# EmilyJrxx/YOLO_PPF_Pose_Estimation

Measured on AMD Instinct MI355X. Metric: PPF pair-matches/sec (accumulator votes) per cropped scene, higher is better.
Workload: dtype u32 votes / f64 pair features

## Files before the change

### yolo_ppf_pose_estimation_amd/csrc/ppf_match_kernels.h

```cpp
#ifndef PPF_MATCH_KERNELS_H
#define PPF_MATCH_KERNELS_H

#ifndef PPF_GUARD_REL
#define PPF_GUARD_REL 5e-7f
#endif
#ifndef PPF_AGG_MIN_HITS
#define PPF_AGG_MIN_HITS 24
#endif
#ifndef PPF_AGG_MIN_RECORDS
#define PPF_AGG_MIN_RECORDS 32
#endif
#ifndef PPF_ABL_COUNTED
#define PPF_ABL_COUNTED 1
#endif
#ifndef PPF_ABL_OWNCELL
#define PPF_ABL_OWNCELL 1
#endif
#ifndef PPF_ABL_DIRECT_SMALL
#define PPF_ABL_DIRECT_SMALL 1
#endif
#ifndef PPF_ABL_DIRECT_BIG
#define PPF_ABL_DIRECT_BIG 1
#endif
#ifndef PPF_MOCK_PAIRBINS
// ... 24 lines not shown
#ifndef PPF_COST_TABLE
#define PPF_COST_TABLE 16
#endif
#ifndef PPF_COST_MIN_HITS
#define PPF_COST_MIN_HITS 8
#endif
#ifndef PPF_COST_ITEM
#define PPF_COST_ITEM 512
#endif
#ifndef PPF_ACC32_COST
#define PPF_ACC32_COST 1.02
#endif
#ifndef PPF_ACC32_SWITCH
#define PPF_ACC32_SWITCH 0.05
#endif
#ifndef PPF_TWO_QUEUES
#define PPF_TWO_QUEUES 0
#endif
#ifndef PPF_PIPE_VALU
#define PPF_PIPE_VALU 4
#endif

constexpr int PAIR_BLOCK = 256;
#ifndef PPF_PAIRS_PER_THREAD
#define PPF_PAIRS_PER_THREAD 12
#endif
constexpr int PAIRS_PER_THREAD = PPF_PAIRS_PER_THREAD;
constexpr int VOTE_BLOCK = 1024;
constexpr int VOTE_WAVES = VOTE_BLOCK / 64;
constexpr int VOTE_UNROLL = 4;
constexpr int VOTE_CHUNK = 64 * VOTE_UNROLL * 4;
constexpr int VOTE_MAX_HITS = PPF_AGG_MIN_HITS;
#ifndef PPF_AGG_CHUNK
#define PPF_AGG_CHUNK 1024
#endif
static_assert(PPF_AGG_CHUNK >= 32 && PPF_AGG_CHUNK % 32 == 0, "chunks of pair records start in different blocks of 32 (MatchArgs::grp_hdr)");
constexpr int AGG_CHUNK = PPF_AGG_CHUNK;
constexpr int AGG_NY = 16;
constexpr int AGG_SUB = 191;
constexpr int AGG_MAX_ANGLES = 31;
#ifndef PPF_RUN_SEG
#define PPF_RUN_SEG 704
#endif
constexpr int RUN_SEG = PPF_RUN_SEG;
constexpr int RUN_SEG_MAX = 1024;
static_assert(RUN_SEG % 64 == 0 && RUN_SEG <= RUN_SEG_MAX && RUN_SEG_MAX == 1024, "the staging area is sized in steps of 64 runs");
constexpr int GROUP_BLOCK = 512;
#ifndef PPF_GROUP_MLP
#define PPF_GROUP_MLP 4
#endif
constexpr int GROUP_MLP = PPF_GROUP_MLP;
constexpr int GROUP_MAX_BUCKETS = 36000;
constexpr int POOL_STRIPES = 64;
constexpr int LDS_HEADER = 256;

constexpr int CUR_STRIDE = 32;
constexpr int CUR_SORTED = POOL_STRIPES * CUR_STRIDE;
constexpr int CUR_RUNS = CUR_SORTED + CUR_STRIDE;
constexpr int CUR_ODDVALUES = CUR_RUNS + CUR_STRIDE;
constexpr int CUR_OVFCOUNT = CUR_ODDVALUES + CUR_STRIDE;
constexpr int CUR_TABLES = CUR_OVFCOUNT + CUR_STRIDE;
constexpr int CUR_OVERFLOW = CUR_TABLES + CUR_STRIDE;
constexpr int CUR_WORDS = CUR_OVERFLOW + CUR_STRIDE;

constexpr int AGG_ROW = 20;
constexpr int AGG_ROW_CE = 17;
constexpr int AGG_SCRATCH = ((AGG_Q + 1) * AGG_ROW + 15) / 16 * 16;
constexpr int AGG_OFF_COLS = (AGG_Q + 1) * AGG_ROW;
constexpr uint32_t AGG_COLS_ALL = (2u << AGG_NY) - 1u;
constexpr int AGG_GROUP_CELLS = 4;
constexpr uint32_t AGG_NARROW_MAX = 255u / AGG_GROUP_CELLS;
constexpr uint32_t AGG_COLS_NARROW = 1u << 31;
constexpr uint32_t AGG_CELLS_FREE = (uint32_t)AGG_Q * 0x01010101u;
constexpr uint32_t AGG_GROUP_X = 8u;
static_assert(AGG_OFF_COLS % 4 == 0 && AGG_OFF_COLS + 4 <= AGG_SCRATCH, "the column mask lives in the padding behind the rows");
constexpr int TBL_OFF_A32 = AGG_SCRATCH;
constexpr int TBL_A32_BYTES = (AGG_NY * AGG_Q > 768 ? AGG_NY * AGG_Q : 768);
constexpr int TBL_OFF_IDX = TBL_OFF_A32 + TBL_A32_BYTES;
constexpr int TBL_BYTES = TBL_OFF_IDX + 192;
constexpr int AGG_OFF_CE = TBL_BYTES;
constexpr int TBL_BUILD_BYTES = AGG_OFF_CE + ((AGG_Q + 1) * 4 + 15) / 16 * 16;
static_assert(AGG_SUB * 4 <= 768 && AGG_SUB <= 192 && AGG_SUB < 256, "table hit range too long");
static_assert(AGG_SCRATCH % 16 == 0 && TBL_BYTES % 16 == 0, "tables are copied 16 bytes at a time");
constexpr int TABLE_BLOCK = 256;
constexpr double TBL_FRAC_MAX = 1.0 / PPF_AGG_MIN_HITS + 1.0 / AGG_SUB;
constexpr double TBL_FRAC_START = 0.02;

__device__ __forceinline__ float acos32_estimate(double x) {
  const double ax = ppf_fabs(x);
  const float xf = (float)ax;
  const float t = fmaxf((float)(1.0 - ax), 0.0f);
  float p = -0.001441536471247673f;
  p = __builtin_fmaf(p, xf, 0.007245631422847509f);
  p = __builtin_fmaf(p, xf, -0.01780921407043934f);
  p = __builtin_fmaf(p, xf, 0.03133561089634895f);
  p = __builtin_fmaf(p, xf, -0.0503128282725811f);
  p = __builtin_fmaf(p, xf, 0.08899927139282227f);
  p = __builtin_fmaf(p, xf, -0.21459989249706268f);
  p = __builtin_fmaf(p, xf, 1.5707963705062866f);
  const float a = __builtin_amdgcn_sqrtf(t) * p;
  return x >= 0.0 ? a : 3.14159274101257324f - a;
}

struct FastKeyConsts {
  float rstep32;
  float gq;
  double rdstep;
};

__device__ __forceinline__ void pair_key(const ppf_vec3& p1, const ppf_vec3& n1, const ppf_vec3& p2, const ppf_vec3& n2,
                                         const double angle_step, const double dist_step, const FastKeyConsts& fk, int32_t (&k)[4]) {
  const double dx = p2.x - p1.x, dy = p2.y - p1.y, dz = p2.z - p1.z;
  const double d2 = __builtin_fma(dz, dz, __builtin_fma(dy, dy, dx * dx));
  const double hd = 0.5 * d2;
  double rinv = __builtin_amdgcn_rsq(d2);
  rinv = rinv * __builtin_fma(-(hd * rinv), rinv, 1.5);
  rinv = rinv * __builtin_fma(-(hd * rinv), rinv, 1.5);
  const double f3 = d2 * rinv;
  const double x0 = __builtin_fma(n1.z, dz, __builtin_fma(n1.y, dy, n1.x * dx)) * rinv;
  const double x1 = __builtin_fma(n2.z, dz, __builtin_fma(n2.y, dy, n2.x * dx)) * rinv;
  const double x2 = __builtin_fma(n1.z, n2.z, __builtin_fma(n1.y, n2.y, n1.x * n2.x));
  bool slow = !(f3 > 2.0 * PPF_EPS) || !(ppf_fabs(x0) <= 1.0 - 1e-12) || !(ppf_fabs(x1) <= 1.0 - 1e-12) || !(ppf_fabs(x2) <= 1.0);
  {
    const float q0 = acos32_estimate(x0) * fk.rstep32, q1 = acos32_estimate(x1) * fk.rstep32,
                q2 = acos32_estimate(x2) * fk.rstep32;
    k[0] = (int)q0; k[1] = (int)q1; k[2] = (int)q2;
    const float lim = 0.5f - fk.gq;
    slow |= (__builtin_fabsf(__builtin_amdgcn_fractf(q0) - 0.5f) > lim) |
            (__builtin_fabsf(__builtin_amdgcn_fractf(q1) - 0.5f) > lim) |
            (__builtin_fabsf(__builtin_amdgcn_fractf(q2) - 0.5f) > lim);
    const double q3 = f3 * fk.rdstep;
    k[3] = (int)q3;
    const double fr3 = q3 - (double)k[3];
    slow |= !(fr3 > 1e-9 && fr3 < 1.0 - 1e-9) || !(q3 < 1.0e5);
  }
  if (slow) {
    double f[4] = {0, 0, 0, 0};
    ppf_pair_feature(p1, n1, p2, n2, f);
    k[0] = ppf_d2i(f[0] / angle_step); k[1] = ppf_d2i(f[1] / angle_step); k[2] = ppf_d2i(f[2] / angle_step);
    k[3] = ppf_d2i(f[3] / dist_step);
  }
}

__device__ __forceinline__ bool pair_key_darboux(const ppf_vec3& p1, const ppf_vec3& n1, const ppf_vec3& p2, const ppf_vec3& n2,
                                                 const double angle_step, const double dist_step, int32_t (&k)[4]) {
  double f[4];
  if (!ppf_pair_feature_darboux(p1, n1, p2, n2, f)) return false;
  k[0] = ppf_floor_key(f[0] / angle_step); k[1] = ppf_floor_key(f[1] / angle_step); k[2] = ppf_floor_key(f[2] / angle_step);
  k[3] = ppf_floor_key(f[3] / dist_step);
  return true;
}

struct MatchArgs {
  CloudSoA surf;
  CloudSoA paired;
  int same_cloud;
  int scene_step, ref_offset, ref_stride;
  int ref_base, n_ref;
  const SlotWord* slotmap;
  uint32_t slot_mask;
  const int32_t* key_lut;
  KeyDims kd;
  const uint32_t* bucket_off;
  int n_buckets;
  const uint4* records;
  int n_tiles, tile_refs, num_angles, n_model;
// ... 718 lines not shown
  const uint32_t before = (quarter >= 1 ? t1 : 0u) + (quarter >= 2 ? t2 : 0u) + (quarter >= 3 ? t3 : 0u);
  const uint32_t tot = __shfl(before + run, 3, 4);
#pragma unroll
  for (int t = 0; t < PER; t++) {
    less[t] += before;
    more[t] = tot - less[t] - c[t];
  }
  const int yy = lane >> 2;
  uint32_t colw;
  {
    unsigned long long o = __ballot(tot != 0u) & 0x1111111111111111ull;
    o = (o | (o >> 3)) & 0x0303030303030303ull;
    o = (o | (o >> 6)) & 0x000F000F000F000Full;
    o = (o | (o >> 12)) & 0x000000FF000000FFull;
    o = (o | (o >> 24)) & 0xFFFFull;
    colw = ((uint32_t)o | ((uint32_t)o << 1)) & AGG_COLS_ALL;
  }
  uint32_t cmax = 0;
#pragma unroll
  for (int t = 0; t < PER; t++) {
    const uint32_t mprev = __shfl_up(more[t], 4);
    const uint32_t v = less[t] + (lane >= 4 ? mprev : 0u);
    const uint32_t p = (uint32_t)(quarter * PER + t);
    lds_st8(ws + p * AGG_ROW + yy, v);
    if (yy == AGG_NY - 1) lds_st8(ws + p * AGG_ROW + AGG_NY, more[t]);
    cmax = max(cmax, yy == AGG_NY - 1 ? max(v, more[t]) : v);
  }
#pragma unroll
  for (int o = 32; o > 0; o >>= 1) cmax = max(cmax, (uint32_t)__shfl_xor((int)cmax, o));
  if (lane == 0) lds_st(ws + AGG_OFF_COLS, colw | (cmax <= AGG_NARROW_MAX ? AGG_COLS_NARROW : 0u));
  wave_lds_fence();
  uint32_t h = lane < AGG_Q ? lds_ld(ws + AGG_OFF_CE + lane * 4) : 0u;
#pragma unroll
  for (int o = 1; o < AGG_Q; o <<= 1) {
    const uint32_t y = __shfl_up(h, o);
    if (lane >= o) h += y;
  }
  wave_lds_fence();
  if (lane < AGG_Q) lds_st(ws + AGG_OFF_CE + lane * 4, h);
  if (lane == 0) lds_st(ws + AGG_OFF_CE + AGG_Q * 4, (uint32_t)ms);
  wave_lds_fence();
#pragma unroll
  for (int t = 0; t < 3; t++) {
    if (cell[t] != 0xFFFFu) {
      const uint32_t pos = lds_add_rtn(ws + AGG_OFF_CE + (cell[t] % (uint32_t)AGG_Q) * 4, 0xFFFFFFFFu) - 1u;
      lds_st(ws + TBL_OFF_A32 + pos * 4, a32[t]);
      lds_st8(ws + TBL_OFF_IDX + pos, (uint32_t)(lane + 64 * t));
    }
  }
  wave_lds_fence();
  if (lane < AGG_Q) {
    const uint2 se = lds_ld2(ws + AGG_OFF_CE + lane * 4);
    lds_st8(ws + lane * AGG_ROW + AGG_ROW_CE, se.x);
    lds_st8(ws + lane * AGG_ROW + AGG_ROW_CE + 1, se.y);
  }
  if (lane == 0) lds_st8(ws + AGG_Q * AGG_ROW + AGG_ROW_CE + 1, (uint32_t)ms);
  wave_lds_fence();
}

__device__ __forceinline__ float vote_guard_band(const int A) {
#ifdef PPF_FORCE_EXACT
  (void)A;
  return 1.0f;
#else
  return PPF_GUARD_REL * (float)A;
#endif
}

__global__ __launch_bounds__(TABLE_BLOCK) void k_tables(MatchArgs a) {
  __shared__ __align__(16) unsigned char tsm[(TABLE_BLOCK / 64) * TBL_BUILD_BYTES];
  const int lane = threadIdx.x & 63;
  const int wave = __builtin_amdgcn_readfirstlane(threadIdx.x >> 6);
  const uint32_t t = blockIdx.x * (TABLE_BLOCK / 64) + (uint32_t)wave;
  if (t >= a.table_cap) return;
  const uint2 d = a.table_desc[t];
  if (d.y == 0u) return;
  const uint32_t ws = (uint32_t)(uintptr_t)(lds_byte*)(tsm + wave * TBL_BUILD_BYTES);
  const int A = a.num_angles;
  const double s64 = (double)A / (4 * PPF_PI);
  const float S = (float)s64, Og = (float)(0.5 * (double)A + (double)vote_guard_band(A));
  table_build(ws, S, Og, s64, a.s_a64 + d.x, (int)d.y, lane);
  const lds_u32x4* src = (const lds_u32x4*)(uintptr_t)ws;
  uint4* __restrict__ dst = reinterpret_cast<uint4*>(a.tables + (size_t)t * TBL_BYTES);
  for (int q = lane; q < TBL_BYTES / 16; q += 64) {
    const u32x4_t v = src[q];
    dst[q] = make_uint4(v.x, v.y, v.z, v.w);
  }
}

__device__ __forceinline__ void agg_cell(const AggConsts& k, const float am, int& X, int& q) {
  const float x = __builtin_fmaf(am, k.S, k.half_a);
  X = (int)x;
  const float qf = __builtin_amdgcn_fractf(x) * (float)AGG_Q;
  q = (int)qf;
  const float fq = __builtin_amdgcn_fractf(qf);
  constexpr float band = 4.7e-6f * (float)AGG_Q;
  const bool near = !(fq > band && fq < 1.0f - band);
  bool one_by_one = am < -3.1415925f;
  if (__builtin_expect(__any(near), 0)) {
    if (near) {
      const double xd = (double)am * k.s64 + k.half_a64;
      const double Xd = __builtin_floor(xd);
      const double qd = (xd - Xd) * (double)AGG_Q;
      const double qfl = __builtin_floor(qd);
      const double fqd = qd - qfl;
      X = (int)Xd;
      q = (int)qfl;
      one_by_one |= !(fqd > 1e-7 && fqd < 1.0 - 1e-7);
    }
  }
  q = one_by_one ? AGG_Q : min(q, AGG_Q - 1);
}

__device__ uint32_t agg_cell_bits(const float am, const int A) {
  if (A > AGG_MAX_ANGLES) return 0u;
  AggConsts k;
  k.s64 = (double)A / (4 * PPF_PI);
  k.S = (float)k.s64;
  k.half_a = 0.5f * (float)A;
  k.half_a64 = 0.5 * (double)A;
  int X, q;
  agg_cell(k, am, X, q);
  return ((uint32_t)X << ROW_X_SHIFT) | ((uint32_t)q << ROW_Q_SHIFT);
}

struct __attribute__((packed, aligned(4))) gl_quad_t { uint32_t x, y, z, w; };
__device__ __forceinline__ uint4 gl_ld4(const uint32_t* __restrict__ p) {
  const gl_quad_t q = *reinterpret_cast<const gl_quad_t*>(p);
  return make_uint4(q.x, q.y, q.z, q.w);
}
__device__ __forceinline__ uint4 gl_ld4_at(const uint32_t* __restrict__ base, const uint32_t w) {
  return gl_ld4(reinterpret_cast<const uint32_t*>(reinterpret_cast<const char*>(base) + w * 4u));
}

__device__ __forceinline__ void agg_own_vote(const AggConsts& k, const uint32_t rz, const uint32_t rw, const float am_a, const float am_b,
                                             const uint32_t oa, const uint32_t ob, const bool da, const bool db, const uint32_t pa,
                                             const uint32_t pb, const uint32_t inc_a, const uint32_t inc_b,
                                             const unsigned char* __restrict__ tbl, const double* __restrict__ g_a64, const uint32_t ha,
                                             const uint32_t hb) {
  const float xa = __builtin_fmaf(am_a, k.S, __uint_as_float(oa)), xb = __builtin_fmaf(am_b, k.S, __uint_as_float(ob));
  int ba = (int)xa, bb = (int)xb;
  const float fa = da ? __builtin_amdgcn_fractf(xa) : 1.0f, fb = db ? __builtin_amdgcn_fractf(xb) : 1.0f;
  if (__builtin_expect(__any(__builtin_fminf(fa, fb) < k.G2), 0)) {
    uint32_t za = rz, zb = rw;
    asm volatile("" : "+v"(za), "+v"(zb));
    if (fa < k.G2) ba = vote_bin_exact_4pi(__uint_as_float(za), g_a64[tbl[TBL_OFF_IDX + ha]], k.A);
    if (fb < k.G2) bb = vote_bin_exact_4pi(__uint_as_float(zb), g_a64[tbl[TBL_OFF_IDX + hb]], k.A);
  }
  if (da) vote_one(pa, ba, inc_a);
  if (db) vote_one(pb, bb, inc_b);
}

struct AggOwn {
  uint32_t wa, wb;
  uint4 oa, ob;
};
__device__ __forceinline__ void agg_own_fetch(const AggConsts& k, const uint4 rec, const unsigned char* __restrict__ tbl, const int ms, AggOwn& o) {
  (void)ms;
  const uint32_t qa = (rec.x >> ROW_Q_SHIFT) & ROW_Q_MASK, qb = (rec.y >> ROW_Q_SHIFT) & ROW_Q_MASK;
  o.wa = lds_ld(k.ws + qa * AGG_ROW + 16);
  o.wb = lds_ld(k.ws + qb * AGG_ROW + 16);
#if PPF_ABL_OWNCELL
  const uint32_t* __restrict__ toff = reinterpret_cast<const uint32_t*>(tbl + TBL_OFF_A32);
  o.oa = gl_ld4_at(toff, __builtin_amdgcn_ubfe(o.wa, 8u, 8u));
  o.ob = gl_ld4_at(toff, __builtin_amdgcn_ubfe(o.wb, 8u, 8u));
#else
  (void)tbl;
#endif
}

__device__ __forceinline__ void agg_cast(const AggConsts& k, const uint32_t va, const uint32_t vb, const bool ha, const bool hb,
                                         const uint32_t (&wa)[5], const uint32_t (&wb)[5], const uint32_t cols) {
  uint32_t sa[4], sb[4];
  {
    const uint32_t sa0 = ha ? k.sel_hi : k.sel_lo, sta = ha ? k.step_hi : k.step_lo;
    const uint32_t sb0 = hb ? k.sel_hi : k.sel_lo, stb = hb ? k.step_hi : k.step_lo;
#pragma unroll
    for (int jj = 0; jj < 4; jj++) { sa[jj] = sa0 + (uint32_t)jj * sta; sb[jj] = sb0 + (uint32_t)jj * stb; }
  }
#if PPF_MOCK_PAIRBINS == 3
  {
    (void)cols;
    const uint32_t va8 = va & ~7u, vb8 = vb & ~7u;
#pragma unroll
    for (int j = 0; j <= AGG_NY; j += 2) {
      const int j1 = j + 1 > AGG_NY ? j : j + 1;
      const unsigned long long da = ((unsigned long long)__builtin_amdgcn_perm(0u, wa[j1 >> 2], sa[j1 & 3]) << 32) | __builtin_amdgcn_perm(0u, wa[j >> 2], sa[j & 3]);
      const unsigned long long db = ((unsigned long long)__builtin_amdgcn_perm(0u, wb[j1 >> 2], sb[j1 & 3]) << 32) | __builtin_amdgcn_perm(0u, wb[j >> 2], sb[j & 3]);
      typedef __attribute__((address_space(3))) unsigned long long lds_u64;
      (void)__hip_atomic_fetch_add((lds_u64*)(uintptr_t)(va8 + (uint32_t)((AGG_NY - j) * 4)), da, __ATOMIC_RELAXED, __HIP_MEMORY_SCOPE_WORKGROUP);
      (void)__hip_atomic_fetch_add((lds_u64*)(uintptr_t)(vb8 + (uint32_t)((AGG_NY - j) * 4)), db, __ATOMIC_RELAXED, __HIP_MEMORY_SCOPE_WORKGROUP);
    }
  }
#elif PPF_MOCK_PAIRBINS
  (void)cols;
#pragma unroll
  for (int j = 0; j <= AGG_NY; j += 2) {
    lds_add(va + (uint32_t)((AGG_NY - j) * 2), __builtin_amdgcn_perm(wa[(j + 1 > AGG_NY ? j : j + 1) >> 2], wa[j >> 2], sa[(j >> 1) & 3]));
    lds_add(vb + (uint32_t)((AGG_NY - j) * 2), __builtin_amdgcn_perm(wb[(j + 1 > AGG_NY ? j : j + 1) >> 2], wb[j >> 2], sb[(j >> 1) & 3]));
  }
#else
  uint32_t cm = cols;
  asm volatile("" : "+s"(cm));
  if (cm == AGG_COLS_ALL) {
#pragma unroll
    for (int j = 0; j <= AGG_NY; j++) {
      lds_add(va + (uint32_t)((AGG_NY - j) * 4), __builtin_amdgcn_perm(0u, wa[j >> 2], sa[j & 3]));
      lds_add(vb + (uint32_t)((AGG_NY - j) * 4), __builtin_amdgcn_perm(0u, wb[j >> 2], sb[j & 3]));
    }
  } else {
#pragma unroll
    for (int j = 0; j <= AGG_NY; j++) {
      if (cm & (1u << j)) {
        lds_add(va + (uint32_t)((AGG_NY - j) * 4), __builtin_amdgcn_perm(0u, wa[j >> 2], sa[j & 3]));
        lds_add(vb + (uint32_t)((AGG_NY - j) * 4), __builtin_amdgcn_perm(0u, wb[j >> 2], sb[j & 3]));
      }
    }
  }
#endif
}

__device__ __forceinline__ void agg_row_add(const uint32_t t, uint32_t (&w)[5]) {
  const uint2 r01 = lds_ld2(t), r23 = lds_ld2(t + 8);
  const uint32_t r4 = lds_ld(t + 16);
  w[0] += r01.x; w[1] += r01.y; w[2] += r23.x; w[3] += r23.y; w[4] += r4 & 0xFFu;
}

__device__ __forceinline__ void agg_group_pair(const AggConsts& k, const uint4 g, const uint32_t cols) {
  static_assert(AGG_GROUP_CELLS == 4, "a group record holds four cell bytes");
  const int Xa = (int)((g.x >> ROW_X_SHIFT) & 31u), Xb = (int)((g.y >> ROW_X_SHIFT) & 31u);
  const uint32_t pa = k.acc_base + (g.x & ROW_OFFSET_MASK), pb = k.acc_base + (g.y & ROW_OFFSET_MASK);
  const bool ha = (g.x & 1u) != 0, hb = (g.y & 1u) != 0;
  uint32_t va = pa + (uint32_t)((Xa - 8) * 4), vb = pb + (uint32_t)((Xb - 8) * 4);
  asm volatile("" : "+v"(va), "+v"(vb));
  uint32_t wa[5] = {0u, 0u, 0u, 0u, 0u}, wb[5] = {0u, 0u, 0u, 0u, 0u};
  agg_row_add(k.ws + (g.z & 0xFFu) * AGG_ROW, wa);
  agg_row_add(k.ws + (g.w & 0xFFu) * AGG_ROW, wb);
  agg_row_add(k.ws + __builtin_amdgcn_ubfe(g.z, 8u, 8u) * AGG_ROW, wa);
  agg_row_add(k.ws + __builtin_amdgcn_ubfe(g.w, 8u, 8u) * AGG_ROW, wb);
  if (__any(((g.z >> 16) != (AGG_CELLS_FREE >> 16)) | ((g.w >> 16) != (AGG_CELLS_FREE >> 16)))) {
    agg_row_add(k.ws + __builtin_amdgcn_ubfe(g.z, 16u, 8u) * AGG_ROW, wa);
    agg_row_add(k.ws + __builtin_amdgcn_ubfe(g.w, 16u, 8u) * AGG_ROW, wb);
    if (__any(((g.z >> 24) != (AGG_CELLS_FREE >> 24)) | ((g.w >> 24) != (AGG_CELLS_FREE >> 24)))) {
      agg_row_add(k.ws + (g.z >> 24) * AGG_ROW, wa);
      agg_row_add(k.ws + (g.w >> 24) * AGG_ROW, wb);
    }
  }
  agg_cast(k, va, vb, ha, hb, wa, wb, cols);
}

template <bool COUNTED>
__device__ __forceinline__ void agg_pair(const AggConsts& k, const uint4 rec, const AggOwn& own, const unsigned char* __restrict__ tbl,
                                         const double* __restrict__ g_a64, const uint32_t cols, uint32_t& votes, const bool live = true) {
  const float am_a = __uint_as_float(rec.z), am_b = __uint_as_float(rec.w);
  const uint32_t a4 = own.wa, b4 = own.wb;
  const uint2 ca = make_uint2(__builtin_amdgcn_ubfe(a4, 8u, 8u), __builtin_amdgcn_ubfe(a4, 16u, 8u));
  const uint2 cb = make_uint2(__builtin_amdgcn_ubfe(b4, 8u, 8u), __builtin_amdgcn_ubfe(b4, 16u, 8u));
  const uint32_t pa = k.acc_base + (rec.x & ROW_OFFSET_MASK), pb = k.acc_base + (rec.y & ROW_OFFSET_MASK);
  const uint32_t inc_a = vote_inc(k.vi, rec.x), inc_b = vote_inc(k.vi, rec.y);
#if !PPF_ABL_COUNTED
  (void)cols;
#else
  if constexpr (COUNTED) {
    const int Xa = (int)((rec.x >> ROW_X_SHIFT) & 31u), qa = (int)((rec.x >> ROW_Q_SHIFT) & ROW_Q_MASK);
    const int Xb = (int)((rec.y >> ROW_X_SHIFT) & 31u), qb = (int)((rec.y >> ROW_Q_SHIFT) & ROW_Q_MASK);
    const uint32_t ta = k.ws + (uint32_t)qa * AGG_ROW, tb = k.ws + (uint32_t)qb * AGG_ROW;
    const uint2 a01 = lds_ld2(ta), a23 = lds_ld2(ta + 8);
    const uint2 b01 = lds_ld2(tb), b23 = lds_ld2(tb + 8);
    const bool ha = (rec.x & 1u) != 0, hb = (rec.y & 1u) != 0;
    uint32_t va = pa + (uint32_t)((Xa - 8) * 4), vb = pb + (uint32_t)((Xb - 8) * 4);
    asm volatile("" : "+v"(va), "+v"(vb));
    const uint32_t wa[5] = {a01.x, a01.y, a23.x, a23.y, a4}, wb[5] = {b01.x, b01.y, b23.x, b23.y, b4};
    agg_cast(k, va, vb, ha, hb, wa, wb, cols);
  }
#endif
  const uint32_t na = live ? ca.y - ca.x : 0u, nb = live ? cb.y - cb.x : 0u;
  votes += na + nb;
#if PPF_ABL_OWNCELL
  if (__any((na > 0u) | (nb > 0u))) {
#define PPF_OWN_VOTE(OA, OB, J) \
    agg_own_vote(k, rec.z, rec.w, am_a, am_b, OA, OB, (J) < na, (J) < nb, pa, pb, inc_a, inc_b, tbl, g_a64, ca.x + (J), cb.x + (J))
    PPF_OWN_VOTE(own.oa.x, own.ob.x, 0u);
    if (__any((1u < na) | (1u < nb))) {
      PPF_OWN_VOTE(own.oa.y, own.ob.y, 1u);
      if (__any((2u < na) | (2u < nb))) {
        PPF_OWN_VOTE(own.oa.z, own.ob.z, 2u);
        if (__any((3u < na) | (3u < nb))) {
          PPF_OWN_VOTE(own.oa.w, own.ob.w, 3u);
          if (__builtin_expect(__any((4u < na) | (4u < nb)), 0)) {
            const uint32_t* __restrict__ toff = reinterpret_cast<const uint32_t*>(tbl + TBL_OFF_A32);
            for (uint32_t done = 4u;;) {
              const uint4 oa = gl_ld4_at(toff, min(ca.x + done, (uint32_t)AGG_SUB)), ob = gl_ld4_at(toff, min(cb.x + done, (uint32_t)AGG_SUB));
              PPF_OWN_VOTE(oa.x, ob.x, done + 0u);
              if (!__any((done + 1u < na) | (done + 1u < nb))) break;
              PPF_OWN_VOTE(oa.y, ob.y, done + 1u);
              if (!__any((done + 2u < na) | (done + 2u < nb))) break;
              PPF_OWN_VOTE(oa.z, ob.z, done + 2u);
              if (!__any((done + 3u < na) | (done + 3u < nb))) break;
              PPF_OWN_VOTE(oa.w, ob.w, done + 3u);
              done += 4u;
              if (!__any((done < na) | (done < nb))) break;
            }
          }
        }
      }
    }
#undef PPF_OWN_VOTE
  }
#endif
}

constexpr int ITEM_C_BITS = 13, ITEM_NH_BITS = 8;
static_assert(VOTE_CHUNK < (1 << ITEM_C_BITS) && AGG_CHUNK < (1 << ITEM_C_BITS) && VOTE_MAX_HITS < (1 << ITEM_NH_BITS) && AGG_SUB < (1 << ITEM_NH_BITS),
              "an item's records and hits share one word of its staged record");
__host__ __device__ constexpr size_t vote_seg_bytes(int run_seg) { return ((size_t)(run_seg + 1) * 24 + 15) / 16 * 16; }
__host__ __device__ constexpr int vote_item_seg(int run_seg) { return (int)(vote_seg_bytes(run_seg) / 16); }
struct VoteItem {
  const uint4* src;
  uint32_t c;
  uint32_t g0;
  int nh;
  bool agg;
  double a64;
  uint4 rec0;
  const unsigned char* tbl;
};

#ifndef PPF_PREFETCH
#define PPF_PREFETCH 2
#endif
__device__ __forceinline__ void vote_fetch_hits(VoteItem& it, const int lane, const MatchArgs& a) {
  it.a64 = (!it.agg && lane < it.nh) ? a.s_a64[it.g0 + lane] : 0.0;
}
__device__ __forceinline__ void vote_fetch_records(VoteItem& it, const int lane) {
  const uint32_t idx = (!it.agg && it.c <= 32) ? ((uint32_t)lane >> 1) : (uint32_t)lane;
  it.rec0 = rec_at(it.src, min(idx, it.c - 1));
}
static_assert(AGG_SCRATCH / 16 <= 128, "the table copy gives a lane two 16-byte pieces");

__device__ __forceinline__ void vote_item_settle(VoteItem& it) {
  uint32_t lo = (uint32_t)__double2loint(it.a64), hi = (uint32_t)__double2hiint(it.a64);
  asm volatile("" : "+v"(lo), "+v"(hi), "+v"(it.rec0.x), "+v"(it.rec0.y), "+v"(it.rec0.z), "+v"(it.rec0.w));
  it.a64 = __hiloint2double((int)hi, (int)lo);
}

struct VoteRun {
  uint32_t off, cnt;
  uint32_t hit0, m;
  uint32_t tbl0;
  uint32_t nchunk;
  uint32_t agg;
};
__device__ __forceinline__ uint4 vote_item_record(const VoteRun& r, const uint32_t sub, const uint32_t chunk) {
  const uint32_t chunk_sz = r.agg ? (uint32_t)AGG_CHUNK : (uint32_t)VOTE_CHUNK;
  const uint32_t group_sz = r.agg ? (uint32_t)AGG_SUB : (uint32_t)VOTE_MAX_HITS;
  const uint32_t c = min(chunk_sz, r.cnt - chunk * chunk_sz), nh = min(group_sz, r.m - sub * group_sz);
  return make_uint4(r.off + chunk * chunk_sz, r.hit0 + sub * group_sz, r.tbl0 + sub, c | (nh << ITEM_C_BITS) | (r.agg << (ITEM_C_BITS + ITEM_NH_BITS)));
}

__device__ __forceinline__ void vote_locate(VoteItem& it, const uint32_t item, const uint4* seg, const int lane, const MatchArgs& a,
                                            const uint4* __restrict__ records) {
  const uint4 rec = seg[item];
  const uint32_t first = (uint32_t)__builtin_amdgcn_readfirstlane((int)rec.x);
  const uint32_t w = (uint32_t)__builtin_amdgcn_readfirstlane((int)rec.w);
  it.g0 = (uint32_t)__builtin_amdgcn_readfirstlane((int)rec.y);
  it.agg = (w >> (ITEM_C_BITS + ITEM_NH_BITS)) != 0;
  it.c = w & ((1u << ITEM_C_BITS) - 1u);
  it.nh = (int)((w >> ITEM_C_BITS) & ((1u << ITEM_NH_BITS) - 1u));
  it.src = records + first;
  it.tbl = it.agg ? a.tables + (size_t)(uint32_t)__builtin_amdgcn_readfirstlane((int)rec.z) * TBL_BYTES : nullptr;
#if PPF_PREFETCH >= 1
  vote_fetch_hits(it, lane, a);
#endif
#if PPF_PREFETCH >= 2
  vote_fetch_records(it, lane);
// ... 14 lines not shown
  uint32_t* acc = lds_acc + GW;

  const int tid = threadIdx.x, lane = tid & 63;
  const int wave = __builtin_amdgcn_readfirstlane(tid >> 6);
  const bool listed = ACC32 && a.acc32 == 2;
  const uint32_t n_work = listed ? 2u * a.cursors[CUR_OVFCOUNT] : gridDim.x;
  uint32_t wid = blockIdx.x;
  if (ACC32 && wid >= n_work) return;
  do {
  int vt, tile, r;
  if (listed) {
    const uint32_t e = a.ovf_list[wid >> 1];
    r = (int)(e & 0xFFFFu);
    tile = (int)(e >> 16);
    vt = 2 * tile + (int)(wid & 1u);
  } else {
    vt = (int)(wid / (uint32_t)a.n_ref);
    tile = ACC32 ? vt >> 1 : vt;
    r = (int)a.perm[wid - (uint32_t)vt * (uint32_t)a.n_ref];
  }
  const int rg = a.ref_base + r;
  const int tile_base = tile * a.tile_refs;
  const int refs_here = min(a.tile_refs, a.n_model - tile_base);
  const int H = (a.tile_refs + 1) >> 1;
  const int words = GW + min(H, refs_here) * P + 1;
  constexpr bool acc32 = ACC32;
  if (tid == 0) { red[50] = red[51] = red[52] = red[53] = red[58] = red[59] = 0u; }

  const uint32_t* __restrict__ boff = a.bucket_off + (size_t)tile * (a.n_buckets + 1);
  if (!ACC32 && a.item_votes) {
    unsigned long long v = 0;
    for (int blk = 0; blk < a.n_rounds; blk++) {
      const uint2 rb = a.run_blocks[(size_t)r * a.n_rounds + blk];
      for (uint32_t i = (uint32_t)tid; i < rb.y; i += VOTE_BLOCK) {
        const uint4 run = a.runs[rb.x + i];
        v += (unsigned long long)run.z * (unsigned long long)(boff[run.x + 1] - boff[run.x]);
      }
    }
#pragma unroll
    for (int o = 32; o > 0; o >>= 1) v += __shfl_down(v, o);
    unsigned long long* red64 = reinterpret_cast<unsigned long long*>(red + 16);
    __syncthreads();
    if (lane == 0) red64[wave] = v;
    __syncthreads();
    unsigned long long V = 0;
#pragma unroll
    for (int k = 0; k < VOTE_WAVES; k++) V += red64[k];
    V *= 2ull;
    const size_t item = (size_t)rg * a.n_tiles + tile;
    if (tid == 0) a.item_votes[item] = V;
    if (V >= a.heavy_votes) {
      if (tid == 0) {
        a.ovf_items[item] = 2u;
        a.ovf_list[atomicAdd(&a.cursors[CUR_OVFCOUNT], 1u)] = (uint32_t)r | ((uint32_t)tile << 16);
      }
      return;
    }
    __syncthreads();
  }
  const uint4* __restrict__ records = a.records;
  const double s64 = WRAP ? (double)A / (2 * PPF_PI) : (double)A / (4 * PPF_PI);
  const float S = (float)s64;
  const float G = WRAP ? fmaxf(1.6e-6f * (float)A, vote_guard_band(A) >= 1.0f ? 1.0f : 0.0f) : vote_guard_band(A);
  const float G2 = 2.0f * G;
  const double og64 = (WRAP ? 1.5 : 0.5) * (double)A + (double)G;
  const uint32_t tail_bytes = (uint32_t)(lane * 4 + 8);
  AggConsts ak;
  ak.acc_base = (uint32_t)(uintptr_t)(lds_byte*)reinterpret_cast<unsigned char*>(lds_acc);
  ak.ws = (uint32_t)(uintptr_t)(lds_byte*)(wave_scratch + wave * AGG_SCRATCH);
  ak.S = S; ak.half_a = 0.5f * (float)A; ak.Og = (float)og64; ak.G2 = G2;
  ak.s64 = s64; ak.half_a64 = 0.5 * (double)A;
  ak.A = A;
  const uint32_t acc_base = ak.acc_base;
  const uint32_t agg_min = (!WRAP && a.agg_min_hits > 0 && A <= AGG_MAX_ANGLES) ? (uint32_t)a.agg_min_hits : 0xFFFFFFFFu;
  unsigned long long ops = 0;
  uint32_t agg_votes = 0;
#ifdef PPF_DIAG_COLUMNS
  unsigned long long diag_dense = 0, diag_cols = 0, diag_full = 0;
#endif
  unsigned long long issued = 0;

  const int pass = ACC32 ? (vt & 1) : 0;
  PPF_PHASE_DECL;
  {
    uint4* z = reinterpret_cast<uint4*>(lds_acc);
    uint32_t zero = 0u;
    asm volatile("" : "+v"(zero));
    for (int c = tid; c < words / 4; c += VOTE_BLOCK) z[c] = make_uint4(zero, zero, zero, zero);
    for (int c = (words & ~3) + tid; c < words; c += VOTE_BLOCK) lds_acc[c] = 0u;
  }
  VoteInc vi;
  vi.lo = acc32 ? (pass == 0 ? 1u : 0u) : 1u;
  vi.hi = acc32 ? (pass == 1 ? 1u : 0u) : 0x10000u;
  ak.vi = vi;
  ak.sel_lo = (acc32 && pass == 1) ? 0x0c0c0c0cu : 0x0c0c0c00u; ak.step_lo = (acc32 && pass == 1) ? 0u : 1u;
  ak.sel_hi = acc32 ? (pass == 1 ? 0x0c0c0c00u : 0x0c0c0c0cu) : 0x0c000c0cu;
  ak.step_hi = acc32 ? (pass == 1 ? 1u : 0u) : 0x10000u;

  for (int blk = 0; blk < a.n_rounds; blk++) {
    const uint2 rb = a.run_blocks[(size_t)r * a.n_rounds + blk];
    uint32_t run_first = 0, item_first = 0;
    while (run_first < rb.y) {
      __syncthreads();
      PPF_PHASE((run_first | item_first) ? 5 : 0);
      const uint32_t n_read = min(min(IS, (uint32_t)VOTE_BLOCK), rb.y - run_first);
      uint32_t items = 0, local0 = 0;
      VoteRun vr;
      vr.off = vr.cnt = vr.hit0 = vr.m = vr.tbl0 = vr.agg = 0u; vr.nchunk = 1u;
      bool heavy_run = false;
      if ((uint32_t)tid < n_read) {
        const uint4 run = a.runs[rb.x + run_first + tid];
        vr.off = boff[run.x];
        vr.cnt = boff[run.x + 1] - vr.off;
        if (acc32) {
          const uint32_t n0 = a.bucket_mid[(size_t)tile * a.n_buckets + run.x], blk = 32u * (n0 >> 6), d = n0 & 63u;
          if (pass == 0) vr.cnt = min(vr.cnt, blk + min(d, 32u));
          else { const uint32_t skip = min(vr.cnt, blk + (d > 32u ? d - 32u : 0u)); vr.off += skip; vr.cnt -= skip; }
        }
        vr.hit0 = run.y;
        vr.m = run.z;
        vr.tbl0 = run.w;
        heavy_run = run.z >= agg_min;
        (void)heavy_run;
        if (vr.cnt) {
          if (run.z >= agg_min && vr.cnt >= PPF_AGG_MIN_RECORDS) {
            vr.nchunk = (vr.cnt + AGG_CHUNK - 1) / AGG_CHUNK;
            items = ((run.z + AGG_SUB - 1) / AGG_SUB) * vr.nchunk;
            vr.agg = 1u;
          } else {
            vr.nchunk = (vr.cnt + VOTE_CHUNK - 1) / VOTE_CHUNK;
            items = ((run.z + VOTE_MAX_HITS - 1) / VOTE_MAX_HITS) * vr.nchunk;
          }
        }
        if (tid == 0) { local0 = item_first; items -= item_first; }
      }
      uint32_t incl = items;
      if constexpr (ACC32) {
#pragma unroll
        for (int o = 1; o < 64; o <<= 1) {
          const uint32_t y = __shfl_up(incl, o);
          if (lane >= o) incl += y;
        }
      } else {
        int lane_s = lane;
        asm volatile("" : "+v"(lane_s));
#pragma unroll
        for (int o = 1; o < 64; o <<= 1) {
          const uint32_t y = (uint32_t)__builtin_amdgcn_ds_bpermute((lane_s - o) << 2, (int)incl);
          if (lane_s >= o) incl += y;
        }
      }
      if (lane == 63) red[wave] = incl;
#if PPF_TWO_QUEUES
      { const uint32_t nh = (uint32_t)__popcll(__ballot(heavy_run)); if (lane == 0) red[16 + wave] = nh; }
#endif
      __syncthreads();
      uint32_t woff = 0, total = 0;
#pragma unroll
      for (int kk = 0; kk < VOTE_WAVES; kk++) {
        const uint32_t w = red[kk];
        if (kk < wave) woff += w;
        total += w;
      }
      const uint32_t first = woff + incl - items;
      const uint32_t n_items = min(total, IS);
      const uint32_t n_mine = first < IS ? min(items, IS - first) : 0u;
      constexpr uint32_t STAGE_OWN = 4;
      if (n_mine) {
        uint32_t sub = local0 / vr.nchunk, chunk = local0 - sub * vr.nchunk;
        for (uint32_t j = 0; j < min(n_mine, STAGE_OWN); j++) {
          seg[first + j] = vote_item_record(vr, sub, chunk);
          if (++chunk == vr.nchunk) { chunk = 0u; sub++; }
        }
      }
      for (unsigned long long many = __ballot(n_mine > STAGE_OWN); many; many &= many - 1ull) {
        const int src = __builtin_ctzll(many);
        VoteRun wr;
        wr.off = (uint32_t)__builtin_amdgcn_readlane((int)vr.off, src); wr.cnt = (uint32_t)__builtin_amdgcn_readlane((int)vr.cnt, src);
        wr.hit0 = (uint32_t)__builtin_amdgcn_readlane((int)vr.hit0, src); wr.m = (uint32_t)__builtin_amdgcn_readlane((int)vr.m, src);
        wr.tbl0 = (uint32_t)__builtin_amdgcn_readlane((int)vr.tbl0, src); wr.nchunk = (uint32_t)__builtin_amdgcn_readlane((int)vr.nchunk, src);
        wr.agg = (uint32_t)__builtin_amdgcn_readlane((int)vr.agg, src);
        const uint32_t w_first = (uint32_t)__builtin_amdgcn_readlane((int)first, src), w_n = (uint32_t)__builtin_amdgcn_readlane((int)n_mine, src);
        const uint32_t w_local0 = (uint32_t)__builtin_amdgcn_readlane((int)local0, src);
        for (uint32_t j = STAGE_OWN + (uint32_t)lane; j < w_n; j += 64u) {
          const uint32_t local = w_local0 + j, sub = local / wr.nchunk;
          seg[w_first + j] = vote_item_record(wr, sub, local - sub * wr.nchunk);
        }
      }
      if (items > IS - first) { red[54] = run_first + (uint32_t)tid; red[55] = local0 + (IS - first); }
#if PPF_TWO_QUEUES
      {
        uint32_t n_heavy = 0;
#pragma unroll
        for (int kk = 0; kk < VOTE_WAVES; kk++) n_heavy += red[16 + kk];
        if (tid == (int)n_heavy && n_heavy < (uint32_t)VOTE_BLOCK) red[56] = min(first, IS);
        if (tid == 0) { if (n_heavy >= (uint32_t)VOTE_BLOCK) red[56] = n_items; red[48] = 0u; }
// ... 30 lines not shown
      uint32_t item = 0;
      int q_item = 0;
      bool have = claim(item, q_item);
      if (have) vote_locate(cur, item, seg, lane, a, records);
      vote_item_settle(cur);
      while (have) {
        uint4 tbl0 = make_uint4(0u, 0u, 0u, 0u), tbl1 = tbl0;
        uint2 grp = make_uint2(0u, 0u);
        if (cur.agg) {
          const uint4* __restrict__ t = reinterpret_cast<const uint4*>(cur.tbl);
          tbl0 = rec_at(t, (uint32_t)min(lane, AGG_SCRATCH / 16 - 1));
          tbl1 = rec_at(t, (uint32_t)min(lane + 64, AGG_SCRATCH / 16 - 1));
          if (!ACC32 && cur.c >= 32u && a.grp_hdr) grp = a.grp_hdr[(uint32_t)(cur.src - records) >> 5];
        }
        const bool have_next = claim(item, q_item);
        if (have_next) vote_locate(nxt, item, seg, lane, a, records);
#else
      uint32_t item = (uint32_t)wave;
      bool have = item < n_items;
      if (have) vote_locate(cur, item, seg, lane, a, records);
      vote_item_settle(cur);
      while (have) {
        uint4 tbl0 = make_uint4(0u, 0u, 0u, 0u), tbl1 = tbl0;
        uint2 grp = make_uint2(0u, 0u);
        if (cur.agg) {
          const uint4* __restrict__ t = reinterpret_cast<const uint4*>(cur.tbl);
          tbl0 = rec_at(t, (uint32_t)min(lane, AGG_SCRATCH / 16 - 1));
          tbl1 = rec_at(t, (uint32_t)min(lane + 64, AGG_SCRATCH / 16 - 1));
          if (!ACC32 && cur.c >= 32u && a.grp_hdr) grp = a.grp_hdr[(uint32_t)(cur.src - records) >> 5];
        }
        item = (uint32_t)__builtin_amdgcn_readfirstlane((int)(lane == 0 ? atomicAdd(&red[48], 1u) : 0u));
        const bool have_next = item < n_items;
        if (have_next) vote_locate(nxt, item, seg, lane, a, records);
#endif
#if PPF_PREFETCH < 1
        vote_fetch_hits(cur, lane, a);
#endif
#if PPF_PREFETCH < 2
        vote_fetch_records(cur, lane);
#endif
        PPF_PHASE(1);
        if (cur.agg) {
          const uint32_t c = cur.c;
          const uint4* __restrict__ src = cur.src;
          uint4 rec_cur = cur.rec0;
          {
            lds_u32x4* w = (lds_u32x4*)(uintptr_t)ak.ws;
            wave_lds_fence();
            if (lane < AGG_SCRATCH / 16) w[lane] = u32x4_t{tbl0.x, tbl0.y, tbl0.z, tbl0.w};
            if (lane + 64 < AGG_SCRATCH / 16) w[lane + 64] = u32x4_t{tbl1.x, tbl1.y, tbl1.z, tbl1.w};
            wave_lds_fence();
          }
          const unsigned char* __restrict__ tbl = cur.tbl;
          const double* __restrict__ g_a64 = a.s_a64 + cur.g0;
          constexpr int cols_piece = AGG_OFF_COLS / 16, cols_word = (AGG_OFF_COLS % 16) / 4;
          const uint4 cols_q = cols_piece < 64 ? tbl0 : tbl1;
          const uint32_t cols_w = (uint32_t)__builtin_amdgcn_readlane((int)(cols_word == 0 ? cols_q.x : cols_word == 1 ? cols_q.y : cols_word == 2 ? cols_q.z : cols_q.w), cols_piece & 63);
          const uint32_t cols = cols_w & AGG_COLS_ALL;
          const bool merged = !ACC32 && a.grp_hdr != nullptr && (cols_w & AGG_COLS_NARROW) != 0u;
          if (merged) {
            const uint32_t gn = (uint32_t)__builtin_amdgcn_readfirstlane((int)grp.y);
            if (PPF_ABL_COUNTED && gn) {
              const uint4* __restrict__ gsrc = a.grp_records + (uint32_t)__builtin_amdgcn_readfirstlane((int)grp.x);
              uint32_t g_code = tail_bytes | (AGG_GROUP_X << ROW_X_SHIFT), g_free = AGG_CELLS_FREE;
              asm volatile("" : "+v"(g_code), "+v"(g_free));
              uint4 g_cur = rec_at(gsrc, min((uint32_t)lane, gn - 1));
              for (uint32_t e0 = 0; e0 < gn; e0 += 64) {
                const uint32_t e = e0 + (uint32_t)lane;
                const uint4 g_n1 = rec_at(gsrc, min(e + 64, gn - 1));
                uint4 g = g_cur;
                if (e >= gn) g = make_uint4(g_code, g_code, g_free, g_free);
                agg_group_pair(ak, g, cols);
                g_cur = g_n1;
              }
            }
            AggOwn own_cur;
            agg_own_fetch(ak, rec_cur, tbl, cur.nh, own_cur);
            uint4 rec_n1 = rec_at(src, min((uint32_t)lane + 64u, c - 1));
            for (uint32_t e0 = 0; e0 < c; e0 += 64) {
              const uint32_t e = e0 + (uint32_t)lane;
              const uint4 rec_n2 = rec_at(src, min(e + 128, c - 1));
              AggOwn own_n1;
              agg_own_fetch(ak, rec_n1, tbl, cur.nh, own_n1);
              agg_pair<false>(ak, rec_cur, own_cur, tbl, g_a64, cols, agg_votes, e < c);
              rec_cur = rec_n1;
              rec_n1 = rec_n2;
              own_cur = own_n1;
            }
            ops += 2u * (uint32_t)__builtin_popcount(cols) * 64u * ((gn + 63u) / 64u);
#ifdef PPF_DIAG_COLUMNS
            diag_dense += 2u * (AGG_NY + 1) * 64u * ((gn + 63u) / 64u);
            diag_cols += 2u * (uint32_t)__builtin_popcount(cols) * 64u * ((gn + 63u) / 64u);
            if (cols == AGG_COLS_ALL) diag_full += 2u * (AGG_NY + 1) * 64u * ((gn + 63u) / 64u);
#endif
            issued += 2ull * c * (uint32_t)cur.nh;
          } else {
          AggOwn own_cur;
          agg_own_fetch(ak, rec_cur, tbl, cur.nh, own_cur);
          uint4 rec_n1 = rec_at(src, min((uint32_t)lane + 64u, c - 1));
          for (uint32_t e0 = 0; e0 < c; e0 += 64) {
            const uint32_t e = e0 + (uint32_t)lane;
            const uint4 rec_n2 = rec_at(src, min(e + 128, c - 1));
            AggOwn own_n1;
            agg_own_fetch(ak, rec_n1, tbl, cur.nh, own_n1);
            uint4 rec = rec_cur;
            if (e >= c) { rec.x = tail_bytes | (rec.x & ~ROW_CODE_MASK); rec.y = tail_bytes | (rec.y & ~ROW_CODE_MASK); }
            agg_pair<true>(ak, rec, own_cur, tbl, g_a64, cols, agg_votes);
            rec_cur = rec_n1;
            rec_n1 = rec_n2;
            own_cur = own_n1;
          }
          ops += 2u * (uint32_t)__builtin_popcount(cols) * 64u * ((c + 63u) / 64u);
#ifdef PPF_DIAG_COLUMNS
          diag_dense += 2u * (AGG_NY + 1) * 64u * ((c + 63u) / 64u);
          diag_cols += 2u * (uint32_t)__builtin_popcount(cols) * 64u * ((c + 63u) / 64u);
          if (cols == AGG_COLS_ALL) diag_full += 2u * (AGG_NY + 1) * 64u * ((c + 63u) / 64u);
#endif
          issued += 128ull * ((c + 63u) / 64u) * (uint32_t)cur.nh;
          }
          PPF_PHASE(2);
        } else {
          const uint32_t c = cur.c;
          const int nh = cur.nh;
          uint4 rec0_reg = cur.rec0;
          asm volatile("" : "+v"(rec0_reg.x), "+v"(rec0_reg.y), "+v"(rec0_reg.z), "+v"(rec0_reg.w));
          const float ohg_v = lane < nh ? (WRAP ? (float)(og64 - cur.a64 * s64) : (float)og64 - (float)cur.a64 * S) : 0.f;
          const double* __restrict__ asd = a.s_a64 + cur.g0;
          const uint4* __restrict__ src = cur.src;
          constexpr uint32_t B = 64 * VOTE_UNROLL;
          const uint32_t nfull = c / B;
          ops += 2ull * 64u * ((c + 63u) / 64u) * (uint32_t)nh;
          issued += 128ull * VOTE_UNROLL * nfull * (uint32_t)nh;
#if PPF_ABL_DIRECT_BIG != 1
          if (c > 32) {
#if PPF_ABL_DIRECT_BIG == 2
            uint4 eb[VOTE_UNROLL];
            for (uint32_t e0 = 0; e0 < c; e0 += 64 * VOTE_UNROLL) {
              load_records<VOTE_UNROLL>(eb, src, min(e0, c > 64u * VOTE_UNROLL ? c - 64u * VOTE_UNROLL : 0u), lane);
#pragma unroll
              for (int u = 0; u < VOTE_UNROLL; u++) asm volatile("" ::"v"(eb[u].x), "v"(eb[u].y), "v"(eb[u].z), "v"(eb[u].w));
            }
#endif
            cur = nxt;
            have = have_next;
            continue;
          }
#endif
          if (c <= 32) {
            const uint32_t e = (uint32_t)lane >> 1;
            const uint4 rr = rec0_reg;
            const uint32_t odd = 0u - ((uint32_t)lane & 1u);
            const uint32_t row_bytes = e < c ? bit_select(odd, rr.x, rr.y) : tail_bytes;
            if (PPF_ABL_DIRECT_SMALL) vote_hits_single<WRAP>(acc_base, vi, row_bytes, bit_select(odd, rr.z, rr.w), S, ohg_v, nh, asd, G2, A);
            issued += 64ull * (uint32_t)nh;
          } else {
            uint32_t e0 = 0;
            if (nfull) {
              uint4 ea[VOTE_UNROLL], eb[VOTE_UNROLL];
              ea[0] = rec0_reg;
#pragma unroll
              for (int u = 1; u < VOTE_UNROLL; u++) ea[u] = rec_at(src, (uint32_t)(u * 64 + lane));
              uint32_t b = 0;
              while (true) {
                load_records<VOTE_UNROLL>(eb, src, min(b + 1, nfull - 1) * B, lane);
                vote_hits<VOTE_UNROLL, WRAP>(acc_base, vi, ea, VOTE_UNROLL, S, ohg_v, nh, asd, G2, A);
                if (++b >= nfull) {
#pragma unroll
                  for (int u = 0; u < VOTE_UNROLL; u++) asm volatile("" ::"v"(eb[u].x), "v"(eb[u].y), "v"(eb[u].z), "v"(eb[u].w));
                  break;
                }
                load_records<VOTE_UNROLL>(ea, src, min(b + 1, nfull - 1) * B, lane);
                vote_hits<VOTE_UNROLL, WRAP>(acc_base, vi, eb, VOTE_UNROLL, S, ohg_v, nh, asd, G2, A);
                if (++b >= nfull) {
#pragma unroll
                  for (int u = 0; u < VOTE_UNROLL; u++) asm volatile("" ::"v"(ea[u].x), "v"(ea[u].y), "v"(ea[u].z), "v"(ea[u].w));
                  break;
                }
              }
              e0 = nfull * B;
            }
            if (e0 < c && c - e0 <= 32) {
              const uint32_t e = e0 + ((uint32_t)lane >> 1);
              const uint4 rr = rec_at(src, min(e, c - 1));
              const uint32_t odd = 0u - ((uint32_t)lane & 1u);
              const uint32_t row_bytes = e < c ? bit_select(odd, rr.x, rr.y) : tail_bytes;
              vote_hits_single<WRAP>(acc_base, vi, row_bytes, bit_select(odd, rr.z, rr.w), S, ohg_v, nh, asd, G2, A);
              issued += 64ull * (uint32_t)nh;
            } else if (e0 < c) {
              uint4 et[VOTE_UNROLL];
#pragma unroll
// ... 124 lines not shown
```

Baseline: 14700 billion.

## Copy only the used table extent and overlap accumulator clear with run fetch

The table builder now writes only the front pieces (scratch rows plus the offsets actually used for the hit count) and the needed index pieces, instead of the whole fixed-size table slot. The agg_pair read-ahead is clamped to the real hit count so it never reads past the written bytes. Separately, in the non-32-bit accumulator path, the LDS accumulator clear is moved after the first run/bucket-offset global loads, and the first barrier is dropped, so the clear overlaps those loads. This trades code complexity and reliance on clamp bounds for less global write traffic and a shorter prologue.

```diff
diff --git a/yolo_ppf_pose_estimation_amd/csrc/ppf_match_kernels.h b/yolo_ppf_pose_estimation_amd/csrc/ppf_match_kernels.h
--- a/yolo_ppf_pose_estimation_amd/csrc/ppf_match_kernels.h
+++ b/yolo_ppf_pose_estimation_amd/csrc/ppf_match_kernels.h
@@ -130,6 +130,20 @@
 constexpr int TBL_BUILD_BYTES = AGG_OFF_CE + ((AGG_Q + 1) * 4 + 15) / 16 * 16;
 static_assert(AGG_SUB * 4 <= 768 && AGG_SUB <= 192 && AGG_SUB < 256, "table hit range too long");
 static_assert(AGG_SCRATCH % 16 == 0 && TBL_BYTES % 16 == 0, "tables are copied 16 bytes at a time");
+#ifndef PPF_UNIT_PROLOGUE
+#define PPF_UNIT_PROLOGUE 1
+#endif
+#ifndef PPF_TABLE_EXTENT
+#define PPF_TABLE_EXTENT 1
+#endif
+__host__ __device__ constexpr int table_front_pieces(int ms) {
+  if (PPF_TABLE_EXTENT == 2) return AGG_SCRATCH / 16;
+  const int want = AGG_SCRATCH / 16 + (ms + 4 + 3) / 4;
+  return want < TBL_OFF_IDX / 16 ? want : TBL_OFF_IDX / 16;
+}
+__host__ __device__ constexpr int table_index_pieces(int ms) { return PPF_TABLE_EXTENT == 2 ? 0 : (ms + 15) / 16; }
+static_assert(TBL_OFF_A32 == AGG_SCRATCH && TBL_OFF_IDX % 16 == 0 && (AGG_SUB + 4) * 4 <= TBL_A32_BYTES + 16 &&
+              table_index_pieces(AGG_SUB) * 16 <= TBL_BYTES - TBL_OFF_IDX, "the offsets' read-ahead ends in written bytes, the index pieces inside the slot");
 constexpr int TABLE_BLOCK = 256;
 constexpr double TBL_FRAC_MAX = 1.0 / PPF_AGG_MIN_HITS + 1.0 / AGG_SUB;
 constexpr double TBL_FRAC_START = 0.02;
@@ -1014,10 +1028,19 @@
   table_build(ws, S, Og, s64, a.s_a64 + d.x, (int)d.y, lane);
   const lds_u32x4* src = (const lds_u32x4*)(uintptr_t)ws;
   uint4* __restrict__ dst = reinterpret_cast<uint4*>(a.tables + (size_t)t * TBL_BYTES);
+#if PPF_TABLE_EXTENT == 0
   for (int q = lane; q < TBL_BYTES / 16; q += 64) {
     const u32x4_t v = src[q];
     dst[q] = make_uint4(v.x, v.y, v.z, v.w);
   }
+#else
+  const int n_front = table_front_pieces((int)d.y), n_all = n_front + table_index_pieces((int)d.y);
+  for (int q = lane; q < n_all; q += 64) {
+    const int piece = q < n_front ? q : q - n_front + TBL_OFF_IDX / 16;
+    const u32x4_t v = src[piece];
+    dst[piece] = make_uint4(v.x, v.y, v.z, v.w);
+  }
+#endif
 }
 
 __device__ __forceinline__ void agg_cell(const AggConsts& k, const float am, int& X, int& q) {
@@ -1183,7 +1206,7 @@
 
 template <bool COUNTED>
 __device__ __forceinline__ void agg_pair(const AggConsts& k, const uint4 rec, const AggOwn& own, const unsigned char* __restrict__ tbl,
-                                         const double* __restrict__ g_a64, const uint32_t cols, uint32_t& votes, const bool live = true) {
+                                         const uint32_t ms, const double* __restrict__ g_a64, const uint32_t cols, uint32_t& votes, const bool live = true) {
   const float am_a = __uint_as_float(rec.z), am_b = __uint_as_float(rec.w);
   const uint32_t a4 = own.wa, b4 = own.wb;
   const uint2 ca = make_uint2(__builtin_amdgcn_ubfe(a4, 8u, 8u), __builtin_amdgcn_ubfe(a4, 16u, 8u));
@@ -1222,7 +1245,7 @@
           if (__builtin_expect(__any((4u < na) | (4u < nb)), 0)) {
             const uint32_t* __restrict__ toff = reinterpret_cast<const uint32_t*>(tbl + TBL_OFF_A32);
             for (uint32_t done = 4u;;) {
-              const uint4 oa = gl_ld4_at(toff, min(ca.x + done, (uint32_t)AGG_SUB)), ob = gl_ld4_at(toff, min(cb.x + done, (uint32_t)AGG_SUB));
+              const uint4 oa = gl_ld4_at(toff, min(ca.x + done, ms)), ob = gl_ld4_at(toff, min(cb.x + done, ms));
               PPF_OWN_VOTE(oa.x, ob.x, done + 0u);
               if (!__any((done + 1u < na) | (done + 1u < nb))) break;
               PPF_OWN_VOTE(oa.y, ob.y, done + 1u);
@@ -1403,13 +1426,17 @@
 
   const int pass = ACC32 ? (vt & 1) : 0;
   PPF_PHASE_DECL;
-  {
+  constexpr bool late_clear = PPF_UNIT_PROLOGUE && !ACC32;
+  auto clear_acc = [&]() {
     uint4* z = reinterpret_cast<uint4*>(lds_acc);
     uint32_t zero = 0u;
     asm volatile("" : "+v"(zero));
-    for (int c = tid; c < words / 4; c += VOTE_BLOCK) z[c] = make_uint4(zero, zero, zero, zero);
-    for (int c = (words & ~3) + tid; c < words; c += VOTE_BLOCK) lds_acc[c] = 0u;
-  }
+    int t = tid;
+    if (late_clear) asm volatile("" : "+v"(t));
+    for (int c = t; c < words / 4; c += VOTE_BLOCK) z[c] = make_uint4(zero, zero, zero, zero);
+    for (int c = (words & ~3) + t; c < words; c += VOTE_BLOCK) lds_acc[c] = 0u;
+  };
+  if (!late_clear || a.n_rounds <= 0) clear_acc();
   VoteInc vi;
   vi.lo = acc32 ? (pass == 0 ? 1u : 0u) : 1u;
   vi.hi = acc32 ? (pass == 1 ? 1u : 0u) : 0x10000u;
@@ -1421,18 +1448,28 @@
   for (int blk = 0; blk < a.n_rounds; blk++) {
     const uint2 rb = a.run_blocks[(size_t)r * a.n_rounds + blk];
     uint32_t run_first = 0, item_first = 0;
+    if (late_clear && blk == 0 && rb.y == 0u) clear_acc();
     while (run_first < rb.y) {
-      __syncthreads();
+      const bool seg0 = late_clear && (blk | (int)run_first | (int)item_first) == 0;
+      if (!seg0) __syncthreads();
       PPF_PHASE((run_first | item_first) ? 5 : 0);
       const uint32_t n_read = min(min(IS, (uint32_t)VOTE_BLOCK), rb.y - run_first);
       uint32_t items = 0, local0 = 0;
       VoteRun vr;
       vr.off = vr.cnt = vr.hit0 = vr.m = vr.tbl0 = vr.agg = 0u; vr.nchunk = 1u;
       bool heavy_run = false;
+      uint4 run = make_uint4(0u, 0u, 0u, 0u);
+      uint32_t b_end = 0;
       if ((uint32_t)tid < n_read) {
-        const uint4 run = a.runs[rb.x + run_first + tid];
+        run = a.runs[rb.x + run_first + tid];
         vr.off = boff[run.x];
-        vr.cnt = boff[run.x + 1] - vr.off;
+        b_end = boff[run.x + 1];
+      }
+      if (seg0) {
+        clear_acc();
+      }
+      if ((uint32_t)tid < n_read) {
+        vr.cnt = b_end - vr.off;
         if (acc32) {
           const uint32_t n0 = a.bucket_mid[(size_t)tile * a.n_buckets + run.x], blk = 32u * (n0 >> 6), d = n0 & 63u;
           if (pass == 0) vr.cnt = min(vr.cnt, blk + min(d, 32u));
@@ -1629,7 +1666,7 @@
               const uint4 rec_n2 = rec_at(src, min(e + 128, c - 1));
               AggOwn own_n1;
               agg_own_fetch(ak, rec_n1, tbl, cur.nh, own_n1);
-              agg_pair<false>(ak, rec_cur, own_cur, tbl, g_a64, cols, agg_votes, e < c);
+              agg_pair<false>(ak, rec_cur, own_cur, tbl, (uint32_t)cur.nh, g_a64, cols, agg_votes, e < c);
               rec_cur = rec_n1;
               rec_n1 = rec_n2;
               own_cur = own_n1;
@@ -1652,7 +1689,7 @@
             agg_own_fetch(ak, rec_n1, tbl, cur.nh, own_n1);
             uint4 rec = rec_cur;
             if (e >= c) { rec.x = tail_bytes | (rec.x & ~ROW_CODE_MASK); rec.y = tail_bytes | (rec.y & ~ROW_CODE_MASK); }
-            agg_pair<true>(ak, rec, own_cur, tbl, g_a64, cols, agg_votes);
+            agg_pair<true>(ak, rec, own_cur, tbl, (uint32_t)cur.nh, g_a64, cols, agg_votes);
             rec_cur = rec_n1;
             rec_n1 = rec_n2;
             own_cur = own_n1;
```

New measurement: 14790 billion (median of 6 runs). About the same (+0.6%).
